# quzefan/LuSh-NeRF

Hardware: AMD Instinct MI355X
Metric: training rays/sec (fwd+bwd), N_samples=64+64 (higher is better)
Workload: dtype f16 MFMA forward (one fp16 plane per operand, fp32 accumulate; render outputs within 3e-5 of the fp32 reference); backward fp16 MFMA (one plane, per-launch power-of-two loss scale), fp32 accumulate; 1 GPU; poster_lushnerf 1xMI355X N_rand=4096/GPU N_samples=64 N_importance=64 blur kernel (DSK/RBK) on, fwd+bwd+Adam, one RCCL all-reduce of the flat gradient (BASELINE config C2); rays_per_gpu=4096, marched_rays_per_gpu=20480, planes_fwd=fp16x1, parallelism=dp1

## Files before the change

### lush_nerf_amd/csrc/lush_march.hip

```cpp
#include "lush_common.h"
#include "lush_host.h"
#include "lush_composite.h"
#include <type_traits>
#include "../../include/lush_march.h"
#include "../../include/lush_subframe.h"
#include "../../include/lush_live_fwd.h"

#include <cmath>
#include <string>

namespace lush {

static thread_local std::string g_err;
int set_error(const char* msg) { g_err = msg; return -1; }
int set_hip_error(hipError_t e, const char* what, const char* file, int line) {
    g_err = std::string(hipGetErrorString(e)) + " in " + what + " at " + file + ":" + std::to_string(line);
    return -2;
}

__device__ __forceinline__ float linspace01(int i, int n) {
    if (n == 1) return 0.f;
    const float step = 1.0f / (float)(n - 1);
    return i < n / 2 ? __fmul_rn(step, (float)i) : __fmaf_rn(-step, (float)(n - 1 - i), 1.0f);
}

__device__ __forceinline__ float zgrid_at(float near, float far, int i, int S, int lindisp) {
    const float t = linspace01(i, S);
    if (!lindisp) return __fadd_rn(__fmul_rn(near, __fsub_rn(1.f, t)), __fmul_rn(far, t));
    return 1.f / __fadd_rn(__fmul_rn(1.f / near, __fsub_rn(1.f, t)), __fmul_rn(1.f / far, t));
// ... 46 lines not shown
    }
    s0 = wave_sum(s0); s1 = wave_sum(s1); s2 = wave_sum(s2); sd = wave_sum(sd); sa = wave_sum(sa);
    if (flags != nullptr) {
        const bool any_dens = __ballot(bad_dens) != 0ull, any_raw = __ballot(bad_raw) != 0ull;
        if (lane == 0) {
            if (c.white_bkgd) { s0 += 1.f - sa; s1 += 1.f - sa; s2 += 1.f - sa; }
            auto bad = [](float v) { return !(fabsf(v) <= 3.402823466e38f); };
            const int w = (bad(s0) || bad(s1) || bad(s2) ? LUSH_FAULT_RGB : 0) | (bad(sd) ? LUSH_FAULT_DEPTH : 0) |
                          (bad(sa) ? LUSH_FAULT_ACC : 0) | (any_dens ? LUSH_FAULT_DENSITY : 0) | (any_raw ? LUSH_FAULT_RAW : 0);
            if (w) atomicOr(flags, w << flag_shift);
            rgb[ray * 3 + 0] = s0; rgb[ray * 3 + 1] = s1; rgb[ray * 3 + 2] = s2;
            depth[ray] = sd; acc[ray] = sa;
        }
        return;
    }
    if (lane == 0) {
        if (c.white_bkgd) { s0 += 1.f - sa; s1 += 1.f - sa; s2 += 1.f - sa; }
        rgb[ray * 3 + 0] = s0; rgb[ray * 3 + 1] = s1; rgb[ray * 3 + 2] = s2;
        depth[ray] = sd; acc[ray] = sa;
    }
}

struct CompBwdExtra { float* block_max; float* zero_buf; long long zero_n; int init_drays; };

template <int SPL>
__global__ __launch_bounds__(RAYS_PER_BLOCK * 64) void composite_bwd_kernel(CompIn c, const float* __restrict__ g_rgb,
        const float* __restrict__ g_depth, const float* __restrict__ g_acc, float* __restrict__ draw,
        float* __restrict__ drays, CompBwdExtra X) {
    const int lane = threadIdx.x & 63;
    if (X.zero_buf != nullptr)
        for (long long i = (long long)blockIdx.x * blockDim.x + threadIdx.x; i < X.zero_n; i += (long long)gridDim.x * blockDim.x) X.zero_buf[i] = 0.f;
    float vmax = 0.f;
  for (int ray = blockIdx.x * RAYS_PER_BLOCK + (threadIdx.x >> 6); ray < c.R; ray += gridDim.x * RAYS_PER_BLOCK) {
    float alpha[SPL], dist[SPL], dens[SPL], gate[SPL], zz[SPL], col[SPL][3], T[SPL], norm;
    comp_load<SPL>(c, ray, lane, alpha, dist, dens, gate, zz, col, norm);
    comp_trans<SPL>(alpha, lane, T);
    float gr[3] = {0.f, 0.f, 0.f};
    if (g_rgb) { gr[0] = g_rgb[ray * 3]; gr[1] = g_rgb[ray * 3 + 1]; gr[2] = g_rgb[ray * 3 + 2]; }
    const float gd = g_depth ? g_depth[ray] : 0.f;
    float ga = g_acc ? g_acc[ray] : 0.f;
    if (c.white_bkgd) ga -= gr[0] + gr[1] + gr[2];
    float G[SPL];
#pragma unroll
    for (int e = 0; e < SPL; ++e) G[e] = gr[0] * col[e][0] + gr[1] * col[e][1] + gr[2] * col[e][2] + gd * zz[e] + ga;
    float Fa = 1.f, Fb = 0.f;
#pragma unroll
    for (int e = SPL - 1; e >= 0; --e) {
        Fb = G[e] * alpha[e] + (1.f - alpha[e]) * Fb;
        Fa = (1.f - alpha[e]) * Fa;
    }
    float Sa = Fa, Sb = Fb;
#pragma unroll
    for (int o = 1; o < 64; o <<= 1) {
        const float ta = __shfl_down(Sa, o, 64), tb = __shfl_down(Sb, o, 64);
        if (lane + o < 64) { Sb = Sa * tb + Sb; Sa = Sa * ta; }
    }
    float tail = __shfl_down(Sb, 1, 64);
    if (lane == 63) tail = 0.f;
    float dnorm = 0.f;
    float sfx = tail;
#pragma unroll
    for (int e = SPL - 1; e >= 0; --e) {
        const int j = lane * SPL + e;
        const float wgt = alpha[e] * T[e];
        float4 o = {0.f, 0.f, 0.f, 0.f};
        if (j < c.S) {
            o.x = wgt * gr[0] * col[e][0] * (1.f - col[e][0]);
            o.y = wgt * gr[1] * col[e][1] * (1.f - col[e][1]);
            o.z = wgt * gr[2] * col[e][2] * (1.f - col[e][2]);
            if (j < c.S - 1) {
                const float dalpha = T[e] * (G[e] - sfx);
                const float om = 1.f - alpha[e];
                o.w = dalpha * dist[e] * om * gate[e];
                const float ddist = dalpha * dens[e] * om;
                dnorm += ddist * (dist[e] / (norm > 0.f ? norm : 1.f));
            }
            *reinterpret_cast<float4*>(draw + ((long long)ray * c.S + j) * 4) = o;
            vmax = fmaxf(fmaxf(vmax, fmaxf(fabsf(o.x), fabsf(o.y))), fmaxf(fabsf(o.z), fabsf(o.w)));
        }
        sfx = G[e] * alpha[e] + (1.f - alpha[e]) * sfx;
    }
    dnorm = wave_sum(dnorm);
    if (drays != nullptr) {
        if (X.init_drays) {
            if (lane < 11) drays[(long long)ray * 11 + lane] = (lane >= 3 && lane < 6 && norm > 0.f) ? dnorm * c.rays[(long long)ray * 11 + lane] / norm : 0.f;
        } else if (lane < 3 && norm > 0.f) {
            drays[(long long)ray * 11 + 3 + lane] += dnorm * c.rays[(long long)ray * 11 + 3 + lane] / norm;
        }
    }
  }
    if (X.block_max != nullptr) {
#pragma unroll
        for (int o = 32; o > 0; o >>= 1) vmax = fmaxf(vmax, __shfl_xor(vmax, o, 64));
        __shared__ float sm[RAYS_PER_BLOCK];
        if (lane == 0) sm[threadIdx.x >> 6] = vmax;
        __syncthreads();
        if (threadIdx.x == 0) {
            float m = 0.f;
#pragma unroll
            for (int i = 0; i < RAYS_PER_BLOCK; ++i) m = fmaxf(m, sm[i]);
            X.block_max[blockIdx.x] = m;
        }
    }
}

__global__ __launch_bounds__(256) void loss_scale_kernel(const float* __restrict__ block_max, int n, float* __restrict__ scale2) {
    float m = 0.f;
    for (int i = threadIdx.x; i < n; i += blockDim.x) {
        const float v = block_max[i];
        m = (v <= 3.402823466e38f) ? fmaxf(m, v) : __int_as_float(0x7f800000);
    }
#pragma unroll
    for (int o = 32; o > 0; o >>= 1) m = fmaxf(m, __shfl_xor(m, o, 64));
    __shared__ float sm[4];
    if ((threadIdx.x & 63) == 0) sm[threadIdx.x >> 6] = m;
    __syncthreads();
    if (threadIdx.x == 0) {
        const float mx = fmaxf(fmaxf(sm[0], sm[1]), fmaxf(sm[2], sm[3]));
        float sc = 1.f;
        if (mx > 0.f && mx < 3.0e38f) {
            int e;
            frexpf(mx, &e);
            sc = ldexpf(1.f, 4 - e);
        }
        scale2[0] = sc;
        scale2[1] = 1.f / sc;
// ... 1042 lines not shown
            gx[c] = *reinterpret_cast<const float4*>(dpts + p * 8);
            gv[c] = *reinterpret_cast<const float4*>(dpts + p * 8 + 4);
            zz[c] = z[p];
            if (!in) { gx[c] = make_float4(0.f, 0.f, 0.f, 0.f); gv[c] = gx[c]; }
        }
#pragma unroll
        for (int c = 0; c < 4; ++c) {
            if (s0 + c * 64 < S) {
                a[0] += gx[c].x; a[1] += gx[c].y; a[2] += gx[c].z;
                a[3] += gx[c].x * zz[c]; a[4] += gx[c].y * zz[c]; a[5] += gx[c].z * zz[c];
                a[6] += gv[c].x; a[7] += gv[c].y; a[8] += gv[c].z;
            }
        }
    }
#pragma unroll
    for (int i = 0; i < 9; ++i) a[i] = wave_sum(a[i]);
    float mine = a[0];
#pragma unroll
    for (int i = 1; i < 9; ++i) mine = lane == i ? a[i] : mine;
    if (lane < 9) atomicAdd(drays + (long long)ray * 11 + (lane < 6 ? lane : lane + 2), mine);
}

constexpr int LIVE_BLK = 1024;
__device__ __forceinline__ bool live_row(const float4 v) { return v.x != 0.f || v.y != 0.f || v.z != 0.f || v.w != 0.f; }

struct LiveByDraw {
    const float4* draw; float4* draw_c;
    __device__ __forceinline__ bool live(int p, float4& v) const { v = draw[p]; return live_row(v); }
    __device__ __forceinline__ void emit(int pos, const float4& v) const { draw_c[pos] = v; }
    __device__ __forceinline__ void pad(int p) const { draw_c[p] = make_float4(0.f, 0.f, 0.f, 0.f); }
};
struct LiveByAlpha {
    const float *raw, *z, *noise; float noise_std, near_mask; int S;
    __device__ __forceinline__ bool live(int p, float4&) const {
        const int ray = p / S, j = p - ray * S;
        if (j == S - 1) return true;
        return comp_gate(comp_pre(raw[(long long)p * 4 + 3], noise, noise_std, ray, S, j), z[p + 1], near_mask);
    }
    __device__ __forceinline__ void emit(int, const float4&) const {}
    __device__ __forceinline__ void pad(int) const {}
};

template <class Pred>
__global__ __launch_bounds__(256) void live_count_kernel(const Pred pred, int P, int* __restrict__ blk) {
    const int p0 = blockIdx.x * LIVE_BLK + threadIdx.x * 4;
    int c = 0;
    float4 v;
#pragma unroll
    for (int k = 0; k < 4; ++k) if (p0 + k < P) c += pred.live(p0 + k, v) ? 1 : 0;
#pragma unroll
    for (int o = 32; o > 0; o >>= 1) c += __shfl_xor(c, o, 64);
    __shared__ int sm[4];
    if ((threadIdx.x & 63) == 0) sm[threadIdx.x >> 6] = c;
    __syncthreads();
    if (threadIdx.x == 0) blk[blockIdx.x] = sm[0] + sm[1] + sm[2] + sm[3];
}
__global__ __launch_bounds__(1024) void live_scan_kernel(int* __restrict__ blk, int nblk, int P, int* __restrict__ cnt) {
    __shared__ int sm[1024];
    int carry = 0;
    for (int b0 = 0; b0 < nblk; b0 += 1024) {
        const int i = b0 + (int)threadIdx.x;
        const int v = i < nblk ? blk[i] : 0;
        sm[threadIdx.x] = v;
        __syncthreads();
        for (int o = 1; o < 1024; o <<= 1) {
            const int a = (int)threadIdx.x >= o ? sm[threadIdx.x - o] : 0;
            __syncthreads();
            sm[threadIdx.x] += a;
            __syncthreads();
        }
        if (i < nblk) blk[i] = carry + sm[threadIdx.x] - v;
        const int tot = sm[1023];
        __syncthreads();
        carry += tot;
    }
    if (threadIdx.x == 0) { cnt[0] = carry; cnt[1] = P; }
}
template <class Pred>
__global__ __launch_bounds__(256) void live_scatter_kernel(const Pred pred, int P, int S, int R, const int* __restrict__ blk_off,
                                                          const int* __restrict__ cnt, int* __restrict__ live_idx, int* __restrict__ ray_start) {
    const int p0 = blockIdx.x * LIVE_BLK + threadIdx.x * 4;
    const int lane = threadIdx.x & 63, w = threadIdx.x >> 6;
    float4 v[4];
    int f[4], c = 0;
#pragma unroll
    for (int k = 0; k < 4; ++k) {
        v[k] = make_float4(0.f, 0.f, 0.f, 0.f);
        f[k] = (p0 + k < P && pred.live(p0 + k, v[k])) ? 1 : 0;
        c += f[k];
    }
    int incl = c;
#pragma unroll
    for (int o = 1; o < 64; o <<= 1) { const int a = __shfl_up(incl, o, 64); if (lane >= o) incl += a; }
    __shared__ int sm[4];
    if (lane == 63) sm[w] = incl;
    __syncthreads();
    int base = blk_off[blockIdx.x];
    for (int i = 0; i < w; ++i) base += sm[i];
    int pos = base + incl - c;
    const int total = cnt[0];
#pragma unroll
    for (int k = 0; k < 4; ++k) {
        const int p = p0 + k;
        if (p < P) {
            if (p % S == 0) ray_start[p / S] = pos;
            if (f[k]) { live_idx[pos] = p; pred.emit(pos, v[k]); ++pos; }
            if (p >= total) pred.pad(p);
        }
    }
    if (blockIdx.x == 0 && threadIdx.x == 0) ray_start[R] = total;
}

__global__ __launch_bounds__(256) void live_gather_kernel(const float4* __restrict__ draw, int P, const int* __restrict__ live_idx,
                                                         const int* __restrict__ list_cnt, float4* __restrict__ draw_c, int* __restrict__ cnt) {
    const int n = list_cnt[0];
    int c = 0;
#pragma unroll
    for (int k = 0; k < LIVE_BLK / 256; ++k) {
        const int i = blockIdx.x * LIVE_BLK + k * 256 + threadIdx.x;
        float4 v = make_float4(0.f, 0.f, 0.f, 0.f);
        if (i < n && i < P) v = draw[live_idx[i]];
        if (i < P) draw_c[i] = v;
        c += live_row(v) ? 1 : 0;
    }
#pragma unroll
    for (int o = 32; o > 0; o >>= 1) c += __shfl_xor(c, o, 64);
    __shared__ int sm[4];
    if ((threadIdx.x & 63) == 0) sm[threadIdx.x >> 6] = c;
    __syncthreads();
    if (threadIdx.x == 0) {
        const int t = sm[0] + sm[1] + sm[2] + sm[3];
// ... 103 lines not shown
    if (threadIdx.x != 0 || blockIdx.x != 0) return;
    st->draw_base += (unsigned long long)n_draw_calls;
    for (int s = 0; s < 3; ++s)
        if ((active_mask >> s) & 1) st->steps[s] += 1;
    st->global_step += 1;
    step_state_derive(st, lrate, decay_steps, b1, b2);
}
__global__ void step_state_init_kernel(StepState* st, unsigned long long draw_base, int global_step, int s0, int s1, int s2,
                                       double lrate, double decay_steps, double b1, double b2) {
    if (threadIdx.x != 0 || blockIdx.x != 0) return;
    st->draw_base = draw_base; st->global_step = global_step;
    st->steps[0] = s0; st->steps[1] = s1; st->steps[2] = s2;
    step_state_derive(st, lrate, decay_steps, b1, b2);
}

}

using namespace lush;
#define S_(s) ((hipStream_t)(s))
#define CHECK_LAUNCH() LUSH_HIP(hipGetLastError())
static inline int cdiv(long long a, long long b) { return (int)((a + b - 1) / b); }

template <class Pred>
static int live_list(const Pred& pred, long long P, int R, int S, int* live_idx, int* ray_start, int* cnt, int* blk, lush_stream_t st) {
    const int nblk = (int)((P + LIVE_BLK - 1) / LIVE_BLK);
    hipLaunchKernelGGL(live_count_kernel<Pred>, dim3(nblk), dim3(256), 0, S_(st), pred, (int)P, blk);
    CHECK_LAUNCH();
    hipLaunchKernelGGL(live_scan_kernel, dim3(1), dim3(1024), 0, S_(st), blk, nblk, (int)P, cnt);
    CHECK_LAUNCH();
    hipLaunchKernelGGL(live_scatter_kernel<Pred>, dim3(nblk), dim3(256), 0, S_(st), pred, (int)P, S, R, (const int*)blk, (const int*)cnt, live_idx, ray_start);
    CHECK_LAUNCH();
    return 0;
}

extern "C" {

const char* lush_last_error(void) { return g_err.c_str(); }
int lush_abi_version(void) { return LUSH_ABI_VERSION; }

int lush_zgrid(const float* rays, int R, int S, int lindisp, const float* t_rand, float* z, lush_stream_t st) {
    if (R <= 0 || S <= 0) return set_error("lush_zgrid: empty");
    hipLaunchKernelGGL(zgrid_kernel, dim3(cdiv((long long)R * S, 256)), dim3(256), 0, S_(st), rays, R, S, lindisp, t_rand, z);
    CHECK_LAUNCH();
    return 0;
}
int lush_zfixed(const float* rays, int R, int S, int index, int lindisp, float* z, lush_stream_t st) {
    if (index < 0 || index >= S) return set_error("lush_zfixed: index out of range");
    hipLaunchKernelGGL(zfixed_kernel, dim3(cdiv(R, 256)), dim3(256), 0, S_(st), rays, R, S, index, lindisp, z);
    CHECK_LAUNCH();
    return 0;
}

int lush_composite_fwd(const float* raw, const float* z, const float* rays, int R, int S, const float* noise,
// ... 3 lines not shown
    if (flag_shift < 0 || flag_shift > 16) return set_error("lush_composite_fwd: flag_shift must be in [0,16]");
    CompIn c{raw, z, rays, noise, R, S, noise_std, near_mask, white_bkgd};
    dim3 g(cdiv(R, RAYS_PER_BLOCK)), b(RAYS_PER_BLOCK * 64);
    if (S <= 64) hipLaunchKernelGGL(composite_fwd_kernel<1>, g, b, 0, S_(st), c, rgb, depth, acc, weights, density, flags, flag_shift);
    else if (S <= 128) hipLaunchKernelGGL(composite_fwd_kernel<2>, g, b, 0, S_(st), c, rgb, depth, acc, weights, density, flags, flag_shift);
    else hipLaunchKernelGGL(composite_fwd_kernel<4>, g, b, 0, S_(st), c, rgb, depth, acc, weights, density, flags, flag_shift);
    CHECK_LAUNCH();
    return 0;
}
static int composite_bwd_blocks(int R) {
    int blocks = cdiv(R, RAYS_PER_BLOCK);
    return blocks > 2048 ? 2048 : blocks;
}
int lush_composite_bwd_blocks(int R) { return R > 0 ? composite_bwd_blocks(R) : 0; }

int lush_composite_bwd(const float* raw, const float* z, const float* rays, int R, int S, const float* noise,
                       float noise_std, float near_mask, int white_bkgd, const float* g_rgb, const float* g_depth,
                       const float* g_acc, float* draw, float* drays, float* block_max, float* zero_buf, long long zero_n,
                       int init_drays, lush_stream_t st) {
    if (S < 2 || S > 256) return set_error("lush_composite_bwd: S must be in [2,256]");
    if (zero_buf != nullptr && zero_n < 0) return set_error("lush_composite_bwd: zero_n must not be negative");
    CompIn c{raw, z, rays, noise, R, S, noise_std, near_mask, white_bkgd};
    const CompBwdExtra x{block_max, zero_buf, zero_buf ? zero_n : 0, init_drays};
    dim3 g(composite_bwd_blocks(R)), b(RAYS_PER_BLOCK * 64);
    if (S <= 64) hipLaunchKernelGGL(composite_bwd_kernel<1>, g, b, 0, S_(st), c, g_rgb, g_depth, g_acc, draw, drays, x);
    else if (S <= 128) hipLaunchKernelGGL(composite_bwd_kernel<2>, g, b, 0, S_(st), c, g_rgb, g_depth, g_acc, draw, drays, x);
    else hipLaunchKernelGGL(composite_bwd_kernel<4>, g, b, 0, S_(st), c, g_rgb, g_depth, g_acc, draw, drays, x);
    CHECK_LAUNCH();
    return 0;
}
int lush_loss_scale(const float* block_max, int n, float* scale2, lush_stream_t st) {
    if (!block_max || n < 1 || !scale2) return set_error("lush_loss_scale: maxima and destination are required");
    hipLaunchKernelGGL(loss_scale_kernel, dim3(1), dim3(256), 0, S_(st), block_max, n, scale2);
    CHECK_LAUNCH();
    return 0;
}

int lush_sample_merge(const float* z, const float* weights, int R, int S, int Ni, const float* u, float* z_out,
                      float* z_samples, float* z_std, int* flags, lush_stream_t st) {
    if (S < 3 || S > 256 || Ni < 1 || S + Ni > SM_MAXN) return set_error("lush_sample_merge: need 3<=S<=256, S+Ni<=512");
    hipLaunchKernelGGL(sample_merge_kernel, dim3(cdiv(R, RAYS_PER_BLOCK)), dim3(RAYS_PER_BLOCK * 64), 0, S_(st), z,
                       weights, R, S, Ni, u, z_out, z_samples, z_std, flags);
    CHECK_LAUNCH();
    return 0;
}

int lush_pack_rays_fwd(const float* rays, int N, int ndc, float cx, float cy, float near, float far, float* batch,
                       lush_stream_t st) {
    hipLaunchKernelGGL(pack_rays_fwd_kernel, dim3(cdiv(N, 256)), dim3(256), 0, S_(st), rays, N, ndc, cx, cy, near, far, batch);
    CHECK_LAUNCH();
// ... 220 lines not shown
int lush_ray_grad_reduce(const float* dpts, const float* z, int R, int S, float* drays, lush_stream_t st) {
    hipLaunchKernelGGL(ray_grad_reduce_kernel, dim3(cdiv(R, RAYS_PER_BLOCK)), dim3(RAYS_PER_BLOCK * 64), 0, S_(st), dpts, z, R, S, drays);
    CHECK_LAUNCH();
    return 0;
}

size_t lush_live_aux_bytes(long long P) { return P > 0 ? (size_t)((P + LIVE_BLK - 1) / LIVE_BLK) * sizeof(int) : 0; }

int lush_live_compact(const float* draw, int R, int S, int* live_idx, float* draw_c, int* ray_start, int* cnt, void* aux, lush_stream_t st) {
    const long long P = (long long)R * S;
    if (R <= 0 || S <= 0 || P >= (1LL << 27)) return set_error("lush_live_compact: 1 .. 2^27 - 1 points");
    if (!draw || !live_idx || !draw_c || !ray_start || !cnt || !aux) return set_error("lush_live_compact: every buffer is required");
    return live_list(LiveByDraw{(const float4*)draw, (float4*)draw_c}, P, R, S, live_idx, ray_start, cnt, (int*)aux, st);
}

int lush_live_list(const float* raw, const float* z, const float* noise, float noise_std, float near_mask, int R, int S,
                   int* live_idx, int* ray_start, int* cnt, void* aux, lush_stream_t st) {
    const long long P = (long long)R * S;
    if (R <= 0 || S <= 0 || P >= (1LL << 27)) return set_error("lush_live_list: 1 .. 2^27 - 1 points");
    if (!raw || !z || !live_idx || !ray_start || !cnt || !aux) return set_error("lush_live_list: raw, z and every output buffer are required");
    return live_list(LiveByAlpha{raw, z, noise, noise_std, near_mask, S}, P, R, S, live_idx, ray_start, cnt, (int*)aux, st);
}

int lush_live_gather(const float* draw, int R, int S, const int* live_idx, const int* list_cnt, float* draw_c, int* cnt, lush_stream_t st) {
    const long long P = (long long)R * S;
    if (R <= 0 || S <= 0 || P >= (1LL << 27)) return set_error("lush_live_gather: 1 .. 2^27 - 1 points");
    if (!draw || !live_idx || !list_cnt || !draw_c || !cnt) return set_error("lush_live_gather: every buffer is required");
    if (hipMemsetAsync(cnt, 0, sizeof(int), S_(st)) != hipSuccess) return set_error("lush_live_gather: hipMemsetAsync failed");
    hipLaunchKernelGGL(live_gather_kernel, dim3(cdiv(P, LIVE_BLK)), dim3(256), 0, S_(st), (const float4*)draw, (int)P, live_idx, list_cnt, (float4*)draw_c, cnt);
    CHECK_LAUNCH();
    return 0;
}

int lush_ray_grad_reduce_live(const float* dpts, const float* z, const int* live_idx, const int* ray_start, int R, float* drays, lush_stream_t st) {
    hipLaunchKernelGGL(ray_grad_reduce_live_kernel, dim3(cdiv(R, RAYS_PER_BLOCK)), dim3(RAYS_PER_BLOCK * 64), 0, S_(st), dpts, z, live_idx, ray_start, R, drays);
    CHECK_LAUNCH();
    return 0;
}

int lush_adam(float* param, const float* grad, float* m, float* v, long long n, float lr, float beta1, float beta2,
              float eps, int step, float grad_scale, lush_stream_t st) {
    if (n <= 0) return 0;
    const float bc1 = (float)(1.0 - pow((double)beta1, (double)step));
    const float bc2s = (float)sqrt(1.0 - pow((double)beta2, (double)step));
    hipLaunchKernelGGL(adam_kernel, dim3(cdiv(n, 256)), dim3(256), 0, S_(st), param, grad, m, v, n, lr, beta1, beta2, eps, bc1, bc2s, grad_scale);
    CHECK_LAUNCH();
// ... 61 lines not shown
```

### lush_nerf_amd/csrc/lush_march_abi.hip

```cpp
#include "lush_common.h"
#include "lush_host.h"
#include "../../include/lush_march.h"
#include "../../include/lush_live_fwd.h"

using namespace lush;

namespace {

inline size_t al256(size_t x) { return (x + 255) & ~(size_t)255; }
inline int nplanes(int c) { return c == PLANES_F16 ? 1 : c; }
inline int stash_code(int pf, int pb) { return pb == 0 ? 0 : (pf == PLANES_F16 ? PLANES_F16 : (pf < nplanes(pb) ? pf : nplanes(pb))); }

struct Layout {
    size_t zc, wc, rawc, pkc, stashc;
    size_t zf, zs, wf, rawf, pkf, stashf;
    size_t pkbc, pkbf;
    size_t draw, dstash, dpts;
    size_t live_idx, draw_c, ray_start, live_cnt, live_aux;
    size_t total;
    size_t stashc_bytes, stashf_bytes;
    bool live;
};

inline bool live_mode(const lush_march_cfg* c) {
    return c->planes_bwd != 0 && !(c->variant & LUSH_VARIANT_DENSE_BWD) &&
           mlp_live_kernels(0, c->planes_fwd, c->planes_bwd, c->variant & LUSH_VARIANT_KERNEL_BITS & ~LUSH_VARIANT_DENSE_BWD);
// ... 85 lines not shown
    if (!layout(cfg, L)) return set_error("lush_march_fwd: bad configuration");
    if (!rays || !coarse || !out || !workspace) return set_error("lush_march_fwd: rays, coarse parameters, outputs and workspace are required");
    const int R = cfg->R, S = cfg->N_samples, Ni = cfg->N_importance, Sf = S + Ni;
    const bool two = Ni > 0;
    if (two && !cfg->same_net && !fine) return set_error("lush_march_fwd: the fine parameters are required");
    if (!out->rgb || !out->depth || !out->acc || !out->density) return set_error("lush_march_fwd: rgb, depth, acc, density outputs are required");
    if (two && (!out->rgb0 || !out->depth0 || !out->acc0 || !out->density0 || !out->z_std)) return set_error("lush_march_fwd: the coarse outputs and z_std are required when N_importance > 0");
    const lush_mlp_params* pfine = cfg->same_net ? coarse : fine;
    char* w = (char*)workspace;
    const int pf = cfg->planes_fwd, var = cfg->variant;
    const int sc = L.live ? 0 : stash_code(pf, cfg->planes_bwd);
    const float* t_rand = draws && cfg->perturb > 0.f ? draws->t_rand : nullptr;
    const float* noise_c = draws && cfg->raw_noise_std > 0.f ? draws->noise_c : nullptr;
    const float* u = draws && cfg->perturb > 0.f ? draws->u : nullptr;
    const float* noise_f = draws && cfg->raw_noise_std > 0.f ? draws->noise_f : nullptr;
    const bool trunk = trunk_form(cfg);
    auto mlp = [&](bool final_pass, const float* z, int Sp, const void* pk, const lush_mlp_params* prm, size_t rawoff, size_t stashoff, const float* noise) -> int {
        float* raw = (float*)(w + rawoff);
        if (!(trunk && final_pass)) return lush_mlp_fwd(0, pf, sc, rays, z, R, Sp, pk, prm, raw, w + stashoff, var, st);
        int* lidx = (int*)(w + L.live_idx);
        int* list_cnt = (int*)(w + L.live_cnt) + LUSH_LIVE_LIST_COUNT_WORD;
        int r = lush_mlp_fwd_trunk(0, pf, rays, z, R, Sp, pk, raw, w + stashoff, var, st);
        if (r) return r;
        r = lush_live_list(raw, z, noise, cfg->raw_noise_std, cfg->near_mask, R, Sp, lidx, (int*)(w + L.ray_start), list_cnt, w + L.live_aux, st);
        if (r) return r;
        return lush_mlp_fwd_live_raw(0, pf, stash_code(pf, cfg->planes_bwd), rays, z, R, Sp, pk, w + stashoff, lidx, list_cnt, raw, var, st);
    };
    float* zc = (float*)(w + L.zc);
    int rc = lush_zgrid(rays, R, S, cfg->lindisp, t_rand, zc, st);
    if (rc) return rc;
    const void* pkc = cfg->packed_coarse;
    if (!pkc) {
        rc = lush_mlp_pack_for(0, pf, coarse, w + L.pkc, cfg->variant, st);
        if (rc) return rc;
        pkc = w + L.pkc;
    }
    rc = mlp(!two, zc, S, pkc, coarse, L.rawc, L.stashc, noise_c);
    if (rc) return rc;
    rc = lush_composite_fwd((const float*)(w + L.rawc), zc, rays, R, S, noise_c, cfg->raw_noise_std, cfg->near_mask, cfg->white_bkgd,
                            two ? out->rgb0 : out->rgb, two ? out->depth0 : out->depth, two ? out->acc0 : out->acc, (float*)(w + L.wc),
                            two ? out->density0 : out->density, flags, two ? LUSH_FAULT_COARSE_SHIFT : 0, st);
    if (rc || !two) return rc;
    float* zf = (float*)(w + L.zf);
    rc = lush_sample_merge(zc, (const float*)(w + L.wc), R, S, Ni, u, zf, (float*)(w + L.zs), out->z_std, flags, st);
    if (rc) return rc;
    const void* pkf = cfg->same_net ? pkc : cfg->packed_fine;
    if (!pkf) {
// ... 13 lines not shown
    Layout L;
    if (!layout(cfg, L)) return set_error("lush_march_bwd: bad configuration");
    if (cfg->planes_bwd == 0) return set_error("lush_march_bwd: the forward ran as inference (planes_bwd = 0): nothing was kept");
    if (!rays || !coarse || !g || !workspace || !drays) return set_error("lush_march_bwd: rays, parameters, output gradients, workspace and drays are required");
    const int R = cfg->R, S = cfg->N_samples, Ni = cfg->N_importance, Sf = S + Ni;
    const bool two = Ni > 0;
    const lush_mlp_params* pfine = cfg->same_net ? coarse : fine;
    const lush_mlp_grads* gfine = cfg->same_net ? g_coarse : g_fine;
    char* w = (char*)workspace;
    const int pf = cfg->planes_fwd, pb = cfg->planes_bwd, sc = stash_code(pf, pb), var = cfg->variant & LUSH_VARIANT_KERNEL_BITS;
    const float* noise_c = draws && cfg->raw_noise_std > 0.f ? draws->noise_c : nullptr;
    const float* noise_f = draws && cfg->raw_noise_std > 0.f ? draws->noise_f : nullptr;
    const bool kept = (cfg->variant & LUSH_MARCH_FWD_LIST_KEPT) && trunk_form(cfg);
    bool first_pass = true;
    struct Scratch { float* draw; char* dstash; float* dpts; };
    const Scratch x{(float*)(w + L.draw), w + L.dstash, (float*)(w + L.dpts)};
    auto chain = [&](const lush_mlp_params* prm, size_t zoff, size_t rawoff, size_t stashoff, const void* pk_ready, size_t pkboff, bool repack,
                     int Sp, const float* noise, const float* g_rgb, const float* g_depth, const float* g_acc, const void* pk_fwd, int slot, bool from_fwd) -> int {
        const float* z = (const float*)(w + zoff);
        float *scale4 = nullptr, *zero_buf = nullptr;
        long long zero_n = 0;
        if (!mlp_dstash_header(0, pb, (long long)R * Sp, x.dstash, &scale4, &zero_buf, &zero_n)) return set_error("lush_march_bwd: bad backward plane code");
        float* block_max = scale4 ? x.dpts : nullptr;
        int rc = lush_composite_bwd((const float*)(w + rawoff), z, rays, R, Sp, noise, cfg->raw_noise_std, cfg->near_mask, cfg->white_bkgd,
                                    g_rgb, g_depth, g_acc, x.draw, drays, block_max, zero_buf, zero_n, first_pass ? 1 : 0, st);
        first_pass = false;
        if (rc) return rc;
        if (scale4) {
            rc = lush_loss_scale(block_max, lush_composite_bwd_blocks(R), scale4, st);
            if (rc) return rc;
        }
        const void* pk = pk_ready;
        if (!pk) {
            if (repack) {
                rc = lush_mlp_pack_for(0, pb, prm, w + pkboff, cfg->variant, st);
                if (rc) return rc;
            }
            pk = w + pkboff;
        }
        if (L.live) {
            int* lidx = (int*)(w + L.live_idx);
            int* lcnt = (int*)(w + L.live_cnt) + 2 * slot;
            float* draw_c = (float*)(w + L.draw_c);
            const int* len = lcnt;
            if (from_fwd) {
                len = (const int*)(w + L.live_cnt) + LUSH_LIVE_LIST_COUNT_WORD;
                rc = lush_live_gather(x.draw, R, Sp, lidx, len, draw_c, lcnt, st);
                if (rc) return rc;
            } else {
                rc = lush_live_compact(x.draw, R, Sp, lidx, draw_c, (int*)(w + L.ray_start), lcnt, w + L.live_aux, st);
                if (rc) return rc;
                const void* pkf = pk_fwd;
                rc = lush_mlp_fwd_live(0, pf, sc, rays, z, R, Sp, pkf, prm, w + stashoff, lidx, lcnt, var, st);
                if (rc) return rc;
            }
            rc = mlp_bwd_chain_prepared(0, sc, pb, rays, z, R, Sp, pk, prm, draw_c, w + stashoff, x.dstash, x.dpts, var, (hipStream_t)st, lidx, len);
            if (rc) return rc;
            return lush_ray_grad_reduce_live(x.dpts, z, lidx, (const int*)(w + L.ray_start), R, drays, st);
        }
        rc = mlp_bwd_chain_prepared(0, sc, pb, rays, z, R, Sp, pk, prm, x.draw, w + stashoff, x.dstash, x.dpts, var, (hipStream_t)st);
        if (rc) return rc;
        return lush_ray_grad_reduce(x.dpts, z, R, Sp, drays, st);
    };
    auto weights = [&](const lush_mlp_params* prm, const lush_mlp_grads* gr, size_t stashoff, int Sp, int slot, bool from_fwd) -> int {
        if (L.live) return mlp_bwd_weights_prepared(0, sc, pb, R, Sp, prm, (const float*)(w + L.draw_c), w + stashoff, x.dstash, gr, var, (hipStream_t)st,
                                                    (const int*)(w + L.live_cnt) + (from_fwd ? LUSH_LIVE_LIST_COUNT_WORD : 2 * slot));
        return mlp_bwd_weights_prepared(0, sc, pb, R, Sp, prm, x.draw, w + stashoff, x.dstash, gr, var, (hipStream_t)st);
    };
    const bool any_main = g->rgb || g->depth || g->acc;
    const bool any_c = two ? (g->rgb0 || g->depth0 || g->acc0) : any_main;
    if ((two && any_main && !gfine) || (any_c && !g_coarse))
        return set_error("lush_march_bwd: gradient buffers of a pass that received output gradients are required");
    int rc = 0;
// ... 22 lines not shown
```

### lush_nerf_amd/lib.py

```python
from __future__ import annotations

import ctypes as C
import os
import subprocess
from typing import Sequence

from . import abi

HERE = os.path.dirname(os.path.abspath(__file__))
CSRC = os.path.join(HERE, "csrc")
SO_PATH = os.path.join(HERE, "liblush_march.so")
SOURCES = ["lush_march.hip", "lush_mlp.hip", "lush_mlp_chain.hip", "lush_mlp_wide.hip", "lush_mlp_wide_bwd.hip", "lush_abi.hip", "lush_march_abi.hip", "lush_field.hip"]
HEADERS = ["lush_common.h", "lush_composite.h", "lush_mlp.h", "lush_mlp_dev.h", "lush_mlp_wide.h", "lush_host.h", os.path.join("..", "..", "include", "lush_live_fwd.h"),
           os.path.join("..", "..", "include", "lush_subframe.h"),
           os.path.join("..", "..", "include", "lush_march.h")]

_lib = None


def _hipcc() -> str:
    for c in (os.environ.get("HIPCC"), "/opt/rocm/bin/hipcc", "hipcc"):
        if c and (os.path.isabs(c) and os.path.exists(c) or not os.path.isabs(c)):
            return c
    return "hipcc"


def needs_build() -> bool:
    if not os.path.exists(SO_PATH):
        return True
    t = os.path.getmtime(SO_PATH)
    return any(os.path.getmtime(os.path.join(CSRC, f)) > t for f in SOURCES + HEADERS)


def use_library(path: str):
    global SO_PATH, _lib
    if _lib is not None:
# ... 57 lines not shown


_abi = abi.parse(open(os.path.join(CSRC, HEADERS[-1])).read())
_SIGS = _abi.protos
EXPORTS = list(_SIGS)
MlpParams, RbkParams = _abi.structs["lush_mlp_params"], _abi.structs["lush_rbk_params"]
MarchCfgC, PackJobC = _abi.structs["lush_march_cfg"], _abi.structs["lush_pack_job"]
MarchDraws, MarchOut, MarchGout = (_abi.structs["lush_march_" + n] for n in ("draws", "out", "gout"))
globals().update({k[len("LUSH_"):]: v for k, v in _abi.consts.items()})
_FAULT_KEYS = {"RGB": ("rgb_map", "rgb0"), "DEPTH": ("depth_map", "depth0"), "ACC": ("acc_map", "acc0"),
               "DENSITY": ("density_map", "density0"), "RAW": ("raw", "raw0")}
FAULT_NAMES = {_abi.consts["LUSH_FAULT_" + c] << shift: keys[k]
               for k, shift in enumerate((0, _abi.consts["LUSH_FAULT_COARSE_SHIFT"])) for c, keys in _FAULT_KEYS.items()}
FAULT_NAMES[_abi.consts["LUSH_FAULT_ZSTD"]] = "z_std"
FAULT_BITS = {n: b for b, n in FAULT_NAMES.items()}
_abi_subframe = abi.parse(open(os.path.join(CSRC, HEADERS[-2])).read(), "lush_subframe.h")
_SIGS_SUBFRAME = _abi_subframe.protos
EXPORTS_SUBFRAME = list(_SIGS_SUBFRAME)
_abi_live_fwd = abi.parse(open(os.path.join(CSRC, HEADERS[-3])).read(), "lush_live_fwd.h")
_SIGS_LIVE_FWD = _abi_live_fwd.protos
EXPORTS_LIVE_FWD = list(_SIGS_LIVE_FWD)
MARCH_FWD_LIST_KEPT = _abi_live_fwd.consts["LUSH_MARCH_FWD_LIST_KEPT"]
LIVE_LIST_COUNT_WORD = _abi_live_fwd.consts["LUSH_LIVE_LIST_COUNT_WORD"]


def fault_names(word: int):
    return [n for b, n in FAULT_NAMES.items() if word & b]


def load():
    global _lib
    if _lib is not None:
        return _lib
    import torch
    if not os.path.exists(SO_PATH):
        raise RuntimeError(f"{SO_PATH} is missing: run `python -c 'import __graft_entry__ as g; g.build()'` "
                           "(the HIP extension is required; there is no fallback path)")
    lib = C.CDLL(SO_PATH)
    for name, (args, res) in (*_SIGS.items(), *_SIGS_SUBFRAME.items(), *_SIGS_LIVE_FWD.items()):
        fn = getattr(lib, name)
        fn.argtypes = args
        fn.restype = res
    _lib = lib
    return lib


def call(name: str, *args):
    lib = load()
    rc = getattr(lib, name)(*args)
    if rc != 0:
        raise RuntimeError(f"{name} failed ({rc}): {lib.lush_last_error().decode()}")


def ptr(t):
    return None if t is None else C.c_void_p(t.data_ptr())


def mlp_struct(tensors: Sequence, n_layers: int) -> MlpParams:
    s = MlpParams()
    for l in range(n_layers):
        s.w[l] = tensors[2 * l].data_ptr()
        s.b[l] = tensors[2 * l + 1].data_ptr()
# ... 19 lines not shown
```

Before: 354,300 rays/s.

## Write composite backward grads straight into compacted live list; bitmask live listing

When the live list comes from the forward pass, the composite backward kernel now computes each sample's position in the compacted list with wave ballots and writes gradients directly into draw_c. This removes the full-size draw write and the separate gather pass. Live-list building now stores per-wave ballot bitmasks in a mark kernel so the place kernel does not re-evaluate the predicate. The block scan is rewritten from a shared-memory Hillis-Steele scan to wave shuffles. The cost is extra ballot work in the backward kernel, a small count-sum launch, and reuse of the dpts buffer as mark scratch, which may alias other data.

```diff
diff --git a/include/lush_live_book.h b/include/lush_live_book.h
--- /dev/null
+++ b/include/lush_live_book.h
@@ -0,0 +1,22 @@
+#ifndef LUSH_LIVE_BOOK_H
+#define LUSH_LIVE_BOOK_H
+#include "lush_march.h"
+
+#ifdef __cplusplus
+extern "C" {
+#endif
+
+size_t lush_live_mark_bytes(long long P);
+int lush_live_list_marked(const float* raw, const float* z, const float* noise, float noise_std, float near_mask, int R, int S,
+                          int* live_idx, int* ray_start, int* cnt, void* aux, void* marks, lush_stream_t stream);
+int lush_live_compact_marked(const float* draw, int R, int S, int* live_idx, float* draw_c, int* ray_start, int* cnt, void* aux,
+                             void* marks, lush_stream_t stream);
+int lush_composite_bwd_listed(const float* raw, const float* z, const float* rays, int R, int S, const float* noise,
+                              float noise_std, float near_mask, int white_bkgd, const float* g_rgb, const float* g_depth,
+                              const float* g_acc, const int* ray_start, const int* list_cnt, float* draw_c, int* cnt, int* blk_cnt,
+                              float* drays, float* block_max, float* zero_buf, long long zero_n, int init_drays, lush_stream_t stream);
+
+#ifdef __cplusplus
+}
+#endif
+#endif
diff --git a/lush_nerf_amd/csrc/lush_march.hip b/lush_nerf_amd/csrc/lush_march.hip
--- a/lush_nerf_amd/csrc/lush_march.hip
+++ b/lush_nerf_amd/csrc/lush_march.hip
@@ -5,6 +5,7 @@
 #include "../../include/lush_march.h"
 #include "../../include/lush_subframe.h"
 #include "../../include/lush_live_fwd.h"
+#include "../../include/lush_live_book.h"
 
 #include <cmath>
 #include <string>
@@ -97,15 +98,26 @@
 }
 
 struct CompBwdExtra { float* block_max; float* zero_buf; long long zero_n; int init_drays; };
-
-template <int SPL>
+__device__ __forceinline__ bool live_row(const float4 v) { return v.x != 0.f || v.y != 0.f || v.z != 0.f || v.w != 0.f; }
+
+struct CompBwdList { float4* draw_c; const int* ray_start; const int* list_cnt; int* blk_cnt; };
+
+template <int SPL, bool LISTED>
 __global__ __launch_bounds__(RAYS_PER_BLOCK * 64) void composite_bwd_kernel(CompIn c, const float* __restrict__ g_rgb,
         const float* __restrict__ g_depth, const float* __restrict__ g_acc, float* __restrict__ draw,
-        float* __restrict__ drays, CompBwdExtra X) {
+        float* __restrict__ drays, CompBwdExtra X, CompBwdList Lst) {
     const int lane = threadIdx.x & 63;
     if (X.zero_buf != nullptr)
         for (long long i = (long long)blockIdx.x * blockDim.x + threadIdx.x; i < X.zero_n; i += (long long)gridDim.x * blockDim.x) X.zero_buf[i] = 0.f;
     float vmax = 0.f;
+    int n_list = 0, nz = 0;
+    if constexpr (LISTED) {
+        const long long P = (long long)c.R * c.S;
+        const int n = Lst.list_cnt[0];
+        n_list = n < 0 ? 0 : (n > P ? (int)P : n);
+        for (long long i = n_list + (long long)blockIdx.x * blockDim.x + threadIdx.x; i < P; i += (long long)gridDim.x * blockDim.x)
+            Lst.draw_c[i] = make_float4(0.f, 0.f, 0.f, 0.f);
+    }
   for (int ray = blockIdx.x * RAYS_PER_BLOCK + (threadIdx.x >> 6); ray < c.R; ray += gridDim.x * RAYS_PER_BLOCK) {
     float alpha[SPL], dist[SPL], dens[SPL], gate[SPL], zz[SPL], col[SPL][3], T[SPL], norm;
     comp_load<SPL>(c, ray, lane, alpha, dist, dens, gate, zz, col, norm);
@@ -134,6 +146,20 @@
     if (lane == 63) tail = 0.f;
     float dnorm = 0.f;
     float sfx = tail;
+    int pos[SPL];
+    if constexpr (LISTED) {
+        const unsigned long long below = (1ull << lane) - 1ull;
+        bool f[SPL];
+        int at = Lst.ray_start[ray];
+#pragma unroll
+        for (int e = 0; e < SPL; ++e) {
+            const int j = lane * SPL + e;
+            f[e] = j < c.S && (j == c.S - 1 || gate[e] != 0.f);
+            at += __popcll(__ballot(f[e]) & below);
+        }
+#pragma unroll
+        for (int e = 0; e < SPL; ++e) { pos[e] = f[e] && at >= 0 && at < n_list ? at : -1; at += f[e] ? 1 : 0; }
+    }
 #pragma unroll
     for (int e = SPL - 1; e >= 0; --e) {
         const int j = lane * SPL + e;
@@ -150,7 +176,11 @@
                 const float ddist = dalpha * dens[e] * om;
                 dnorm += ddist * (dist[e] / (norm > 0.f ? norm : 1.f));
             }
-            *reinterpret_cast<float4*>(draw + ((long long)ray * c.S + j) * 4) = o;
+            if constexpr (LISTED) {
+                if (pos[e] >= 0) { Lst.draw_c[pos[e]] = o; nz += live_row(o) ? 1 : 0; }
+            } else {
+                *reinterpret_cast<float4*>(draw + ((long long)ray * c.S + j) * 4) = o;
+            }
             vmax = fmaxf(fmaxf(vmax, fmaxf(fabsf(o.x), fabsf(o.y))), fmaxf(fabsf(o.z), fabsf(o.w)));
         }
         sfx = G[e] * alpha[e] + (1.f - alpha[e]) * sfx;
@@ -177,6 +207,29 @@
             X.block_max[blockIdx.x] = m;
         }
     }
+    if constexpr (LISTED) {
+#pragma unroll
+        for (int o = 32; o > 0; o >>= 1) nz += __shfl_xor(nz, o, 64);
+        __shared__ int smc[RAYS_PER_BLOCK];
+        if (lane == 0) smc[threadIdx.x >> 6] = nz;
+        __syncthreads();
+        if (threadIdx.x == 0) {
+            int t = 0;
+#pragma unroll
+            for (int i = 0; i < RAYS_PER_BLOCK; ++i) t += smc[i];
+            Lst.blk_cnt[blockIdx.x] = t;
+        }
+    }
+}
+__global__ __launch_bounds__(256) void live_count_sum_kernel(const int* __restrict__ blk_cnt, int n, int P, int* __restrict__ cnt) {
+    int c = 0;
+    for (int i = threadIdx.x; i < n; i += blockDim.x) c += blk_cnt[i];
+#pragma unroll
+    for (int o = 32; o > 0; o >>= 1) c += __shfl_xor(c, o, 64);
+    __shared__ int sm[4];
+    if ((threadIdx.x & 63) == 0) sm[threadIdx.x >> 6] = c;
+    __syncthreads();
+    if (threadIdx.x == 0) { cnt[0] = sm[0] + sm[1] + sm[2] + sm[3]; cnt[1] = P; }
 }
 
 __global__ __launch_bounds__(256) void loss_scale_kernel(const float* __restrict__ block_max, int n, float* __restrict__ scale2) {
@@ -1265,12 +1318,13 @@
 }
 
 constexpr int LIVE_BLK = 1024;
-__device__ __forceinline__ bool live_row(const float4 v) { return v.x != 0.f || v.y != 0.f || v.z != 0.f || v.w != 0.f; }
+constexpr int LIVE_WORDS = LIVE_BLK / 64;
 
 struct LiveByDraw {
     const float4* draw; float4* draw_c;
     __device__ __forceinline__ bool live(int p, float4& v) const { v = draw[p]; return live_row(v); }
     __device__ __forceinline__ void emit(int pos, const float4& v) const { draw_c[pos] = v; }
+    __device__ __forceinline__ void place(int pos, int p) const { draw_c[pos] = draw[p]; }
     __device__ __forceinline__ void pad(int p) const { draw_c[p] = make_float4(0.f, 0.f, 0.f, 0.f); }
 };
 struct LiveByAlpha {
@@ -1281,6 +1335,7 @@
         return comp_gate(comp_pre(raw[(long long)p * 4 + 3], noise, noise_std, ray, S, j), z[p + 1], near_mask);
     }
     __device__ __forceinline__ void emit(int, const float4&) const {}
+    __device__ __forceinline__ void place(int, int) const {}
     __device__ __forceinline__ void pad(int) const {}
 };
 
@@ -1299,23 +1354,23 @@
     if (threadIdx.x == 0) blk[blockIdx.x] = sm[0] + sm[1] + sm[2] + sm[3];
 }
 __global__ __launch_bounds__(1024) void live_scan_kernel(int* __restrict__ blk, int nblk, int P, int* __restrict__ cnt) {
-    __shared__ int sm[1024];
+    __shared__ int wsum[16];
+    const int lane = threadIdx.x & 63, w = threadIdx.x >> 6;
     int carry = 0;
     for (int b0 = 0; b0 < nblk; b0 += 1024) {
         const int i = b0 + (int)threadIdx.x;
         const int v = i < nblk ? blk[i] : 0;
-        sm[threadIdx.x] = v;
+        int incl = v;
+#pragma unroll
+        for (int o = 1; o < 64; o <<= 1) { const int a = __shfl_up(incl, o, 64); if (lane >= o) incl += a; }
+        if (lane == 63) wsum[w] = incl;
         __syncthreads();
-        for (int o = 1; o < 1024; o <<= 1) {
-            const int a = (int)threadIdx.x >= o ? sm[threadIdx.x - o] : 0;
-            __syncthreads();
-            sm[threadIdx.x] += a;
-            __syncthreads();
-        }
-        if (i < nblk) blk[i] = carry + sm[threadIdx.x] - v;
-        const int tot = sm[1023];
+        int before = 0, tot = 0;
+#pragma unroll
+        for (int k = 0; k < 16; ++k) { const int s = wsum[k]; tot += s; before += k < w ? s : 0; }
+        if (i < nblk) blk[i] = carry + before + incl - v;
+        carry += tot;
         __syncthreads();
-        carry += tot;
     }
     if (threadIdx.x == 0) { cnt[0] = carry; cnt[1] = P; }
 }
@@ -1350,6 +1405,50 @@
             if (f[k]) { live_idx[pos] = p; pred.emit(pos, v[k]); ++pos; }
             if (p >= total) pred.pad(p);
         }
+    }
+    if (blockIdx.x == 0 && threadIdx.x == 0) ray_start[R] = total;
+}
+
+template <class Pred>
+__global__ __launch_bounds__(256) void live_mark_kernel(const Pred pred, int P, int* __restrict__ blk, unsigned long long* __restrict__ marks) {
+    const int lane = threadIdx.x & 63, w = threadIdx.x >> 6;
+    int c = 0;
+    float4 v;
+#pragma unroll
+    for (int k = 0; k < LIVE_WORDS / 4; ++k) {
+        const int word = w * (LIVE_WORDS / 4) + k;
+        const int p = blockIdx.x * LIVE_BLK + word * 64 + lane;
+        const bool f = p < P && pred.live(p, v);
+        const unsigned long long b = __ballot(f);
+        if (lane == 0) marks[(long long)blockIdx.x * LIVE_WORDS + word] = b;
+        c += __popcll(b);
+    }
+    __shared__ int sm[4];
+    if (lane == 0) sm[w] = c;
+    __syncthreads();
+    if (threadIdx.x == 0) blk[blockIdx.x] = sm[0] + sm[1] + sm[2] + sm[3];
+}
+template <class Pred>
+__global__ __launch_bounds__(256) void live_place_kernel(const Pred pred, int P, int S, int R, const int* __restrict__ blk_off, const int* __restrict__ cnt,
+                                                        const unsigned long long* __restrict__ marks, int* __restrict__ live_idx, int* __restrict__ ray_start) {
+    const int lane = threadIdx.x & 63, w = threadIdx.x >> 6;
+    const unsigned long long* m = marks + (long long)blockIdx.x * LIVE_WORDS;
+    int base = blk_off[blockIdx.x];
+    for (int i = 0; i < w * (LIVE_WORDS / 4); ++i) base += __popcll(m[i]);
+    const int total = cnt[0];
+    const unsigned long long below = (1ull << lane) - 1ull;
+#pragma unroll
+    for (int k = 0; k < LIVE_WORDS / 4; ++k) {
+        const int word = w * (LIVE_WORDS / 4) + k;
+        const unsigned long long b = m[word];
+        const int p = blockIdx.x * LIVE_BLK + word * 64 + lane;
+        if (p < P) {
+            const int pos = base + __popcll(b & below);
+            if (p % S == 0) ray_start[p / S] = pos;
+            if ((b >> lane) & 1ull) { live_idx[pos] = p; pred.place(pos, p); }
+            if (p >= total) pred.pad(p);
+        }
+        base += __popcll(b);
     }
     if (blockIdx.x == 0 && threadIdx.x == 0) ray_start[R] = total;
 }
@@ -1499,13 +1598,17 @@
 static inline int cdiv(long long a, long long b) { return (int)((a + b - 1) / b); }
 
 template <class Pred>
-static int live_list(const Pred& pred, long long P, int R, int S, int* live_idx, int* ray_start, int* cnt, int* blk, lush_stream_t st) {
+static int live_list(const Pred& pred, long long P, int R, int S, int* live_idx, int* ray_start, int* cnt, int* blk, lush_stream_t st,
+                     void* marks = nullptr) {
     const int nblk = (int)((P + LIVE_BLK - 1) / LIVE_BLK);
-    hipLaunchKernelGGL(live_count_kernel<Pred>, dim3(nblk), dim3(256), 0, S_(st), pred, (int)P, blk);
+    unsigned long long* mk = (unsigned long long*)marks;
+    if (mk) hipLaunchKernelGGL(live_mark_kernel<Pred>, dim3(nblk), dim3(256), 0, S_(st), pred, (int)P, blk, mk);
+    else hipLaunchKernelGGL(live_count_kernel<Pred>, dim3(nblk), dim3(256), 0, S_(st), pred, (int)P, blk);
     CHECK_LAUNCH();
     hipLaunchKernelGGL(live_scan_kernel, dim3(1), dim3(1024), 0, S_(st), blk, nblk, (int)P, cnt);
     CHECK_LAUNCH();
-    hipLaunchKernelGGL(live_scatter_kernel<Pred>, dim3(nblk), dim3(256), 0, S_(st), pred, (int)P, S, R, (const int*)blk, (const int*)cnt, live_idx, ray_start);
+    if (mk) hipLaunchKernelGGL(live_place_kernel<Pred>, dim3(nblk), dim3(256), 0, S_(st), pred, (int)P, S, R, (const int*)blk, (const int*)cnt, (const unsigned long long*)mk, live_idx, ray_start);
+    else hipLaunchKernelGGL(live_scatter_kernel<Pred>, dim3(nblk), dim3(256), 0, S_(st), pred, (int)P, S, R, (const int*)blk, (const int*)cnt, live_idx, ray_start);
     CHECK_LAUNCH();
     return 0;
 }
@@ -1555,10 +1658,31 @@
     if (zero_buf != nullptr && zero_n < 0) return set_error("lush_composite_bwd: zero_n must not be negative");
     CompIn c{raw, z, rays, noise, R, S, noise_std, near_mask, white_bkgd};
     const CompBwdExtra x{block_max, zero_buf, zero_buf ? zero_n : 0, init_drays};
+    const CompBwdList none{nullptr, nullptr, nullptr, nullptr};
     dim3 g(composite_bwd_blocks(R)), b(RAYS_PER_BLOCK * 64);
-    if (S <= 64) hipLaunchKernelGGL(composite_bwd_kernel<1>, g, b, 0, S_(st), c, g_rgb, g_depth, g_acc, draw, drays, x);
-    else if (S <= 128) hipLaunchKernelGGL(composite_bwd_kernel<2>, g, b, 0, S_(st), c, g_rgb, g_depth, g_acc, draw, drays, x);
-    else hipLaunchKernelGGL(composite_bwd_kernel<4>, g, b, 0, S_(st), c, g_rgb, g_depth, g_acc, draw, drays, x);
+    if (S <= 64) hipLaunchKernelGGL((composite_bwd_kernel<1, false>), g, b, 0, S_(st), c, g_rgb, g_depth, g_acc, draw, drays, x, none);
+    else if (S <= 128) hipLaunchKernelGGL((composite_bwd_kernel<2, false>), g, b, 0, S_(st), c, g_rgb, g_depth, g_acc, draw, drays, x, none);
+    else hipLaunchKernelGGL((composite_bwd_kernel<4, false>), g, b, 0, S_(st), c, g_rgb, g_depth, g_acc, draw, drays, x, none);
+    CHECK_LAUNCH();
+    return 0;
+}
+int lush_composite_bwd_listed(const float* raw, const float* z, const float* rays, int R, int S, const float* noise,
+                              float noise_std, float near_mask, int white_bkgd, const float* g_rgb, const float* g_depth,
+                              const float* g_acc, const int* ray_start, const int* list_cnt, float* draw_c, int* cnt, int* blk_cnt, float* drays,
+                              float* block_max, float* zero_buf, long long zero_n, int init_drays, lush_stream_t st) {
+    if (S < 2 || S > 256) return set_error("lush_composite_bwd_listed: S must be in [2,256]");
+    if (R <= 0 || (long long)R * S >= (1LL << 27)) return set_error("lush_composite_bwd_listed: 1 .. 2^27 - 1 points");
+    if (zero_buf != nullptr && zero_n < 0) return set_error("lush_composite_bwd_listed: zero_n must not be negative");
+    if (!ray_start || !list_cnt || !draw_c || !cnt || !blk_cnt) return set_error("lush_composite_bwd_listed: the list's ranges and length, draw_c, cnt and blk_cnt are required");
+    CompIn c{raw, z, rays, noise, R, S, noise_std, near_mask, white_bkgd};
+    const CompBwdExtra x{block_max, zero_buf, zero_buf ? zero_n : 0, init_drays};
+    const CompBwdList l{(float4*)draw_c, ray_start, list_cnt, blk_cnt};
+    dim3 g(composite_bwd_blocks(R)), b(RAYS_PER_BLOCK * 64);
+    if (S <= 64) hipLaunchKernelGGL((composite_bwd_kernel<1, true>), g, b, 0, S_(st), c, g_rgb, g_depth, g_acc, (float*)nullptr, drays, x, l);
+    else if (S <= 128) hipLaunchKernelGGL((composite_bwd_kernel<2, true>), g, b, 0, S_(st), c, g_rgb, g_depth, g_acc, (float*)nullptr, drays, x, l);
+    else hipLaunchKernelGGL((composite_bwd_kernel<4, true>), g, b, 0, S_(st), c, g_rgb, g_depth, g_acc, (float*)nullptr, drays, x, l);
+    CHECK_LAUNCH();
+    hipLaunchKernelGGL(live_count_sum_kernel, dim3(1), dim3(256), 0, S_(st), (const int*)blk_cnt, (int)g.x, R * S, cnt);
     CHECK_LAUNCH();
     return 0;
 }
@@ -1825,6 +1949,23 @@
     return live_list(LiveByAlpha{raw, z, noise, noise_std, near_mask, S}, P, R, S, live_idx, ray_start, cnt, (int*)aux, st);
 }
 
+size_t lush_live_mark_bytes(long long P) { return P > 0 ? (size_t)((P + LIVE_BLK - 1) / LIVE_BLK) * LIVE_WORDS * sizeof(unsigned long long) : 0; }
+
+int lush_live_compact_marked(const float* draw, int R, int S, int* live_idx, float* draw_c, int* ray_start, int* cnt, void* aux, void* marks, lush_stream_t st) {
+    const long long P = (long long)R * S;
+    if (R <= 0 || S <= 0 || P >= (1LL << 27)) return set_error("lush_live_compact_marked: 1 .. 2^27 - 1 points");
+    if (!draw || !live_idx || !draw_c || !ray_start || !cnt || !aux || !marks) return set_error("lush_live_compact_marked: every buffer is required");
+    return live_list(LiveByDraw{(const float4*)draw, (float4*)draw_c}, P, R, S, live_idx, ray_start, cnt, (int*)aux, st, marks);
+}
+
+int lush_live_list_marked(const float* raw, const float* z, const float* noise, float noise_std, float near_mask, int R, int S,
+                          int* live_idx, int* ray_start, int* cnt, void* aux, void* marks, lush_stream_t st) {
+    const long long P = (long long)R * S;
+    if (R <= 0 || S <= 0 || P >= (1LL << 27)) return set_error("lush_live_list_marked: 1 .. 2^27 - 1 points");
+    if (!raw || !z || !live_idx || !ray_start || !cnt || !aux || !marks) return set_error("lush_live_list_marked: raw, z, every output buffer and the scratch are required");
+    return live_list(LiveByAlpha{raw, z, noise, noise_std, near_mask, S}, P, R, S, live_idx, ray_start, cnt, (int*)aux, st, marks);
+}
+
 int lush_live_gather(const float* draw, int R, int S, const int* live_idx, const int* list_cnt, float* draw_c, int* cnt, lush_stream_t st) {
     const long long P = (long long)R * S;
     if (R <= 0 || S <= 0 || P >= (1LL << 27)) return set_error("lush_live_gather: 1 .. 2^27 - 1 points");
diff --git a/lush_nerf_amd/csrc/lush_march_abi.hip b/lush_nerf_amd/csrc/lush_march_abi.hip
--- a/lush_nerf_amd/csrc/lush_march_abi.hip
+++ b/lush_nerf_amd/csrc/lush_march_abi.hip
@@ -2,6 +2,7 @@
 #include "lush_host.h"
 #include "../../include/lush_march.h"
 #include "../../include/lush_live_fwd.h"
+#include "../../include/lush_live_book.h"
 
 using namespace lush;
 
@@ -133,7 +134,8 @@
         int* list_cnt = (int*)(w + L.live_cnt) + LUSH_LIVE_LIST_COUNT_WORD;
         int r = lush_mlp_fwd_trunk(0, pf, rays, z, R, Sp, pk, raw, w + stashoff, var, st);
         if (r) return r;
-        r = lush_live_list(raw, z, noise, cfg->raw_noise_std, cfg->near_mask, R, Sp, lidx, (int*)(w + L.ray_start), list_cnt, w + L.live_aux, st);
+        r = lush_live_list_marked(raw, z, noise, cfg->raw_noise_std, cfg->near_mask, R, Sp, lidx, (int*)(w + L.ray_start), list_cnt, w + L.live_aux,
+                                  w + L.dpts, st);
         if (r) return r;
         return lush_mlp_fwd_live_raw(0, pf, stash_code(pf, cfg->planes_bwd), rays, z, R, Sp, pk, w + stashoff, lidx, list_cnt, raw, var, st);
     };
@@ -193,8 +195,12 @@
         long long zero_n = 0;
         if (!mlp_dstash_header(0, pb, (long long)R * Sp, x.dstash, &scale4, &zero_buf, &zero_n)) return set_error("lush_march_bwd: bad backward plane code");
         float* block_max = scale4 ? x.dpts : nullptr;
-        int rc = lush_composite_bwd((const float*)(w + rawoff), z, rays, R, Sp, noise, cfg->raw_noise_std, cfg->near_mask, cfg->white_bkgd,
-                                    g_rgb, g_depth, g_acc, x.draw, drays, block_max, zero_buf, zero_n, first_pass ? 1 : 0, st);
+        const bool listed = L.live && from_fwd;
+        int rc = listed ? lush_composite_bwd_listed((const float*)(w + rawoff), z, rays, R, Sp, noise, cfg->raw_noise_std, cfg->near_mask, cfg->white_bkgd,
+                                                    g_rgb, g_depth, g_acc, (const int*)(w + L.ray_start), (const int*)(w + L.live_cnt) + LUSH_LIVE_LIST_COUNT_WORD,
+                                                    (float*)(w + L.draw_c), (int*)(w + L.live_cnt) + 2 * slot, (int*)x.draw, drays, block_max, zero_buf, zero_n, first_pass ? 1 : 0, st)
+                        : lush_composite_bwd((const float*)(w + rawoff), z, rays, R, Sp, noise, cfg->raw_noise_std, cfg->near_mask, cfg->white_bkgd,
+                                             g_rgb, g_depth, g_acc, x.draw, drays, block_max, zero_buf, zero_n, first_pass ? 1 : 0, st);
         first_pass = false;
         if (rc) return rc;
         if (scale4) {
@@ -216,10 +222,8 @@
             const int* len = lcnt;
             if (from_fwd) {
                 len = (const int*)(w + L.live_cnt) + LUSH_LIVE_LIST_COUNT_WORD;
-                rc = lush_live_gather(x.draw, R, Sp, lidx, len, draw_c, lcnt, st);
-                if (rc) return rc;
             } else {
-                rc = lush_live_compact(x.draw, R, Sp, lidx, draw_c, (int*)(w + L.ray_start), lcnt, w + L.live_aux, st);
+                rc = lush_live_compact_marked(x.draw, R, Sp, lidx, draw_c, (int*)(w + L.ray_start), lcnt, w + L.live_aux, x.dpts, st);
                 if (rc) return rc;
                 const void* pkf = pk_fwd;
                 rc = lush_mlp_fwd_live(0, pf, sc, rays, z, R, Sp, pkf, prm, w + stashoff, lidx, lcnt, var, st);
diff --git a/lush_nerf_amd/lib.py b/lush_nerf_amd/lib.py
--- a/lush_nerf_amd/lib.py
+++ b/lush_nerf_amd/lib.py
@@ -11,7 +11,8 @@
 CSRC = os.path.join(HERE, "csrc")
 SO_PATH = os.path.join(HERE, "liblush_march.so")
 SOURCES = ["lush_march.hip", "lush_mlp.hip", "lush_mlp_chain.hip", "lush_mlp_wide.hip", "lush_mlp_wide_bwd.hip", "lush_abi.hip", "lush_march_abi.hip", "lush_field.hip"]
-HEADERS = ["lush_common.h", "lush_composite.h", "lush_mlp.h", "lush_mlp_dev.h", "lush_mlp_wide.h", "lush_host.h", os.path.join("..", "..", "include", "lush_live_fwd.h"),
+HEADERS = ["lush_common.h", "lush_composite.h", "lush_mlp.h", "lush_mlp_dev.h", "lush_mlp_wide.h", "lush_host.h", os.path.join("..", "..", "include", "lush_live_book.h"),
+           os.path.join("..", "..", "include", "lush_live_fwd.h"),
            os.path.join("..", "..", "include", "lush_subframe.h"),
            os.path.join("..", "..", "include", "lush_march.h")]
 
@@ -115,6 +116,9 @@
 EXPORTS_LIVE_FWD = list(_SIGS_LIVE_FWD)
 MARCH_FWD_LIST_KEPT = _abi_live_fwd.consts["LUSH_MARCH_FWD_LIST_KEPT"]
 LIVE_LIST_COUNT_WORD = _abi_live_fwd.consts["LUSH_LIVE_LIST_COUNT_WORD"]
+_abi_live_book = abi.parse(open(os.path.join(CSRC, HEADERS[-4])).read(), "lush_live_book.h")
+_SIGS_LIVE_BOOK = _abi_live_book.protos
+EXPORTS_LIVE_BOOK = list(_SIGS_LIVE_BOOK)
 
 
 def fault_names(word: int):
@@ -130,7 +134,7 @@
         raise RuntimeError(f"{SO_PATH} is missing: run `python -c 'import __graft_entry__ as g; g.build()'` "
                            "(the HIP extension is required; there is no fallback path)")
     lib = C.CDLL(SO_PATH)
-    for name, (args, res) in (*_SIGS.items(), *_SIGS_SUBFRAME.items(), *_SIGS_LIVE_FWD.items()):
+    for name, (args, res) in (*_SIGS.items(), *_SIGS_SUBFRAME.items(), *_SIGS_LIVE_FWD.items(), *_SIGS_LIVE_BOOK.items()):
         fn = getattr(lib, name)
         fn.argtypes = args
         fn.restype = res
```

Result: no change. 356,900 rays/s (median of 6 runs) (+0.7%).
